# OpenVVC/VVCSoftware_VTM

Hardware: AMD Instinct MI355X
Metric: encoded frames/sec (bit-exact bitstream) at 4K10 RA QP32, 1/2/4/8 GPU [M1: hot-path pictures/s of the kernels behind the call sites, NOT EncoderApp fps] (higher is better)
Workload: dtype int16

## Files before the change

### vvcsoftware_vtm_amd/csrc/fracsearch.hip

```cpp
#include "common.h"
#include "mfma_tr.h"
#include "frac_dev.h"

namespace {

__global__ __launch_bounds__(256) void frac_refine_kernel(const Pel* __restrict__ org, int os, const Pel* __restrict__ ref, int rs,
                                                          const vvcgpu_frac_blk* __restrict__ blocks, int nblocks, int w, int h,
                                                          int bd, int cmin, int cmax, int useHad, vvcgpu_mvcost mv,
                                                          const int* __restrict__ preds, int groups,
                                                          int groupBytes, vvcgpu_frac_result* __restrict__ results)
{
  extern __shared__ __align__(16) unsigned char smem[];
  const int gsz = 256 / groups, grp = threadIdx.x / gsz, tid = threadIdx.x - grp * gsz;
  const int b = blockIdx.x * groups + grp;
  const bool active = b < nblocks;
  const int wp = w + 9 + 1;
  const int WR = h + 9;
  unsigned char* base = smem + (size_t)grp * groupBytes;
  FracLds L;
  L.cost = reinterpret_cast<unsigned long long*>(base);
  L.sel = reinterpret_cast<int*>(base + 512);
  L.org = reinterpret_cast<short*>(base + 544);
  L.win = L.org + ((w * h + 7) & ~7);
  L.hpl = L.win + ((wp * WR + 7) & ~7);
  L.pred = L.hpl + ((w * (h + 8) + 7) & ~7);

  vvcgpu_frac_blk blk = { 0, 0, 0, 0, 0, 0 };
  if (active)
  {
    blk = blocks[b];
    if (preds) { mv.pred_hor = preds[2 * b]; mv.pred_ver = preds[2 * b + 1]; }
    const Pel* o = org + (size_t)blk.org_y * os + blk.org_x;
    for (int i = tid; i < w * h; i += gsz) { const int y = i / w, x = i - y * w; L.org[i] = o[(size_t)y * os + x]; }
    const Pel* r0 = ref + (ptrdiff_t)(blk.ref_y - 4) * rs + blk.ref_x - 4;
    for (int i = tid; i < (w + 9) * WR; i += gsz) { const int y = i / (w + 9), x = i - y * (w + 9); L.win[y * wp + x] = r0[(ptrdiff_t)y * rs + x]; }
  }
  frac_refine_pu(L, w, h, wp, bd, cmin, cmax, useHad, mv, blk.mv_x, blk.mv_y, active, tid, gsz, results + (active ? b : 0));
}

template <int CTRL> __device__ __forceinline__ int dpp_mov(int v) { return __builtin_amdgcn_update_dpp(0, v, CTRL, 0xF, 0xF, false); }
constexpr int DPP_XOR1 = 0xB1, DPP_XOR2 = 0x4E, DPP_HALF_MIRROR = 0x141, DPP_ROR8 = 0x128;

template <int CTRL>
__device__ __forceinline__ void had_cross(int (&v)[4], bool upper)
{
#pragma unroll
  for (int j = 0; j < 4; j++) { const int p = dpp_mov<CTRL>(v[j]); v[j] = (upper ? -v[j] : v[j]) + p; }
}

template <bool HAD>
__device__ __forceinline__ unsigned f16_dist(const int (&orgv)[4], const int (&pred)[4], int lane, bool wide)
{
  int d[4];
#pragma unroll
  for (int j = 0; j < 4; j++) d[j] = orgv[j] - pred[j];
  int s;
  if (HAD && wide)
  {
    int v[4] = { d[0] + d[1], d[0] - d[1], d[2] + d[3], d[2] - d[3] };
    { const int a0 = v[0] + v[2], a2 = v[0] - v[2], a1 = v[1] + v[3], a3 = v[1] - v[3]; v[0] = a0; v[1] = a1; v[2] = a2; v[3] = a3; }
    had_cross<DPP_ROR8>(v, (lane & 8) != 0);
    had_cross<DPP_XOR1>(v, (lane & 1) != 0);
    had_cross<DPP_XOR2>(v, (lane & 2) != 0);
#pragma unroll
    for (int j = 0; j < 4; j++)
    {
      int p = __builtin_amdgcn_update_dpp(0, v[j], 0x104, 0xF, 0x5, false);
      p = __builtin_amdgcn_update_dpp(p, v[j], 0x114, 0xF, 0xA, false);
      v[j] = ((lane & 4) ? -v[j] : v[j]) + p;
    }
    s = abs(v[0]) + abs(v[1]) + abs(v[2]) + abs(v[3]);
  }
  else if (HAD)
  {
    const pel2 one = { 1, 1 }, mone = { -1, -1 }, pm = { 1, -1 };
    pel2 q0 = { (short)d[0], (short)d[1] }, q1 = { (short)d[2], (short)d[3] };
    auto rot = [](pel2 v) { const unsigned u = __builtin_bit_cast(unsigned, v); return __builtin_bit_cast(pel2, __builtin_amdgcn_alignbit(u, u, 16)); };
    q0 = rot(q0) + q0 * pm;
    q1 = rot(q1) + q1 * pm;
    { const pel2 a = q0 + q1, b = q0 - q1; q0 = a; q1 = b; }
    auto cross = [&](auto mov, bool upper)
    {
      const pel2 sg = upper ? mone : one;
      q0 = __builtin_bit_cast(pel2, mov(__builtin_bit_cast(int, q0))) + q0 * sg;
      q1 = __builtin_bit_cast(pel2, mov(__builtin_bit_cast(int, q1))) + q1 * sg;
    };
    cross([](int v) { return dpp_mov<DPP_ROR8>(v); }, (lane & 8) != 0);
    cross([](int v) { return dpp_mov<DPP_XOR1>(v); }, (lane & 1) != 0);
    cross([](int v) { return dpp_mov<DPP_XOR2>(v); }, (lane & 2) != 0);
    auto xor4 = [](int v)
    {
      int p = __builtin_amdgcn_update_dpp(0, v, 0x104, 0xF, 0x5, false);
      return __builtin_amdgcn_update_dpp(p, v, 0x114, 0xF, 0xA, false);
    };
    const pel2 a0 = __builtin_elementwise_max(q0, -q0), a1 = __builtin_elementwise_max(q1, -q1);
    const pel2 m0 = __builtin_elementwise_max(a0, __builtin_bit_cast(pel2, xor4(__builtin_bit_cast(int, a0))));
    const pel2 m1 = __builtin_elementwise_max(a1, __builtin_bit_cast(pel2, xor4(__builtin_bit_cast(int, a1))));
    s = (int)m0[0] + (int)m0[1] + (int)m1[0] + (int)m1[1];
  }
  else
    s = abs(d[0]) + abs(d[1]) + abs(d[2]) + abs(d[3]);
  s += dpp_mov<DPP_XOR1>(s); s += dpp_mov<DPP_XOR2>(s); s += dpp_mov<DPP_HALF_MIRROR>(s); s += dpp_mov<DPP_ROR8>(s);
  unsigned t0 = (unsigned)__builtin_amdgcn_readlane(s, 0), t1 = (unsigned)__builtin_amdgcn_readlane(s, 16),
           t2 = (unsigned)__builtin_amdgcn_readlane(s, 32), t3 = (unsigned)__builtin_amdgcn_readlane(s, 48);
  if (HAD) return ((t0 + 2) >> 2) + ((t1 + 2) >> 2) + ((t2 + 2) >> 2) + ((t3 + 2) >> 2);
  return t0 + t1 + t2 + t3;
}

constexpr int HPT = 24;
struct F16Col { unsigned D[6], E[5]; };
__device__ __forceinline__ void f16_load_col(const short* __restrict__ pcT, F16Col& c)
{
  const uint2* q = reinterpret_cast<const uint2*>(pcT);
#pragma unroll
  for (int m = 0; m < 3; m++) { const uint2 v = q[m]; c.D[2 * m] = v.x; c.D[2 * m + 1] = v.y; }
#pragma unroll
  for (int m = 0; m < 5; m++) c.E[m] = __builtin_amdgcn_alignbit(c.D[m + 1], c.D[m], 16);
}

template <int IY>
__device__ __forceinline__ void f16_vert(const F16Col& col, int fy, int headRoom, int cmin, int cmax, int (&out)[4])
{
  if (fy == 0)
  {
#pragma unroll
    for (int yy = 0; yy < 4; yy++)
    {
      const unsigned d = col.D[2 + (yy >> 1)];
      const int v = (yy & 1) ? (int)d >> 16 : (int)(short)(d & 0xFFFF);
      out[yy] = clip3(cmin, cmax, (int)(short)((v + OFFS + (1 << (headRoom - 1))) >> headRoom));
    }
    return;
  }
  const unsigned* cf = reinterpret_cast<const unsigned*>(c_lumaF[fy << 2]);
  const int shift2 = 6 + headRoom, off2 = (1 << (shift2 - 1)) + (OFFS << 6);
  int sum[4] = { off2, off2, off2, off2 };
#pragma unroll
  for (int m = 0; m < 4; m++)
  {
    const pel2 cm = __builtin_bit_cast(pel2, cf[m]);
    if (IY < 0)
    {
      sum[0] = __builtin_amdgcn_sdot2(__builtin_bit_cast(pel2, col.D[m]), cm, sum[0], false);
      sum[1] = __builtin_amdgcn_sdot2(__builtin_bit_cast(pel2, col.E[m]), cm, sum[1], false);
      sum[2] = __builtin_amdgcn_sdot2(__builtin_bit_cast(pel2, col.D[m + 1]), cm, sum[2], false);
      sum[3] = __builtin_amdgcn_sdot2(__builtin_bit_cast(pel2, col.E[m + 1]), cm, sum[3], false);
    }
    else
    {
      sum[0] = __builtin_amdgcn_sdot2(__builtin_bit_cast(pel2, col.E[m]), cm, sum[0], false);
      sum[1] = __builtin_amdgcn_sdot2(__builtin_bit_cast(pel2, col.D[m + 1]), cm, sum[1], false);
      sum[2] = __builtin_amdgcn_sdot2(__builtin_bit_cast(pel2, col.E[m + 1]), cm, sum[2], false);
      sum[3] = __builtin_amdgcn_sdot2(__builtin_bit_cast(pel2, col.D[m + 2]), cm, sum[3], false);
    }
  }
#pragma unroll
  for (int yy = 0; yy < 4; yy++) out[yy] = clip3(cmin, cmax, (int)(short)(sum[yy] >> shift2));
}

template <bool WIDE>
__device__ __forceinline__ void f16_hplane(const short* __restrict__ win, short* __restrict__ hpT, int ix, int fx, int headRoom, int lane)
{
  if (lane < 48)
  {
    const int r = lane >> 1, seg = lane & 1;
    const unsigned* wr = reinterpret_cast<const unsigned*>(win + r * 26 + seg * 8);
    unsigned D[8], E[7];
#pragma unroll
    for (int k = 0; k < 8; k++) D[k] = wr[k];
#pragma unroll
    for (int k = 0; k < 7; k++) E[k] = __builtin_amdgcn_alignbit(D[k + 1], D[k], 16);
    short* o = hpT + (1 + seg * 8) * HPT + r;
    const int shift1 = 6 - headRoom, off1 = -(OFFS << shift1);
    const unsigned* cf = reinterpret_cast<const unsigned*>(c_lumaF[fx << 2]);
    pel2 c2[4];
#pragma unroll
    for (int m = 0; m < 4; m++) c2[m] = __builtin_bit_cast(pel2, cf[m]);
    auto tap8 = [&](int st) -> int
    {
      int sum = off1;
#pragma unroll
      for (int m = 0; m < 4; m++)
        sum = __builtin_amdgcn_sdot2(__builtin_bit_cast(pel2, (st & 1) ? E[(st >> 1) + m] : D[(st >> 1) + m]), c2[m], sum, false);
      return sum >> shift1;
    };
    if (WIDE)
    {
      if (seg == 0)
      {
#pragma unroll
        for (int x = -1; x < 8; x++) o[x * HPT] = (short)tap8(x + 1);
      }
      else
      {
#pragma unroll
        for (int x = 0; x < 8; x++) o[x * HPT] = (short)tap8(x + 1);
      }
    }
    else if (fx == 0)
    {
#pragma unroll
      for (int x = 0; x < 8; x++)
      {
        const unsigned d = D[(x + 4) >> 1];
        const int sv = (x & 1) ? (int)d >> 16 : (int)(short)(d & 0xFFFF);
        o[x * HPT] = (short)((short)(sv << headRoom) - (short)OFFS);
      }
    }
    else if (ix == 0)
    {
#pragma unroll
      for (int x = 0; x < 8; x++) o[x * HPT] = (short)tap8(x + 1);
    }
    else
    {
#pragma unroll
      for (int x = 0; x < 8; x++) o[x * HPT] = (short)tap8(x);
    }
  }
}

#define WAVE_SYNC() do { __builtin_amdgcn_fence(__ATOMIC_ACQ_REL, "wavefront"); __builtin_amdgcn_wave_barrier(); } while (0)

__device__ __forceinline__ int f16_idx(int dx, int dy, bool quarter)
{
  if (dx == 0) return dy == 0 ? 0 : dy < 0 ? 1 : 2;
  if (!quarter) return dx < 0 ? (dy == 0 ? 3 : dy < 0 ? 5 : 7) : (dy == 0 ? 4 : dy < 0 ? 6 : 8);
  return dx < 0 ? (dy < 0 ? 3 : dy == 0 ? 5 : 7) : (dy < 0 ? 4 : dy == 0 ? 6 : 8);
}

__device__ __forceinline__ void f16_best(const unsigned* dist, bool quarter, const vvcgpu_mvcost& mv, int baseX, int baseY, int scale,
                                         int lane, int& bdx, int& bdy, unsigned long long& bcost, unsigned& bdist)
{
  const int li = lane < 9 ? lane : 0;
  const int dx = quarter ? c_refQ[li][0] : c_refH[li][0], dy = quarter ? c_refQ[li][1] : c_refH[li][1];
  const unsigned dl = dist[li];
  unsigned long long c = lane < 9 ? (unsigned long long)dl + mv_cost(mv.lambda, mv.pred_hor, mv.pred_ver, scale, baseX + dx, baseY + dy) : ~0ull;
  int bi = lane;
#pragma unroll
  for (int o = 1; o < 16; o <<= 1)
  {
    const unsigned long long oc = __shfl_xor(c, o);
    const int oi = __shfl_xor(bi, o);
    if (oc < c || (oc == c && oi < bi)) { c = oc; bi = oi; }
  }
  bi = __builtin_amdgcn_readfirstlane(bi);
  bcost = ((unsigned long long)(unsigned)__builtin_amdgcn_readfirstlane((int)(c >> 32)) << 32) | (unsigned)__builtin_amdgcn_readfirstlane((int)c);
  bdx = quarter ? c_refQ[bi][0] : c_refH[bi][0];
  bdy = quarter ? c_refQ[bi][1] : c_refH[bi][1];
  bdist = dist[bi];
}

struct F16Lds { short win[24 * 26]; short hpl[3][24 * 18]; unsigned dist[16]; };

template <bool HAD>
__device__ __forceinline__ void frac16_pu_valu(F16Lds& L, const Pel* __restrict__ org, int os, const Pel* __restrict__ ref, int rs,
                                               const vvcgpu_frac_blk& blk, int b, int bd, int cmin, int cmax, const vvcgpu_mvcost& mv,
                                               vvcgpu_frac_result* __restrict__ results, int lane)
{
  short* win = L.win;
  short* hp0 = L.hpl[0];
  short* hp8 = L.hpl[1];
  short* hpq = L.hpl[2];
  const int t = lane >> 4, x = 8 * (t & 1) + (lane & 7), y0 = 8 * (t >> 1) + 4 * ((lane >> 3) & 1);
  int orgv[4];
  {
    const Pel* o = org + (size_t)(blk.org_y + y0) * os + blk.org_x + x;
#pragma unroll
    for (int j = 0; j < 4; j++) orgv[j] = o[(size_t)j * os];
    const Pel* r0 = ref + (ptrdiff_t)(blk.ref_y - 4) * rs + blk.ref_x - 4;
#pragma unroll
    for (int u = 0; u < 9; u++)
    {
      const int i = lane + 64 * u, r = (i * 2731) >> 16, cc = i - r * 24;
      win[r * 26 + cc] = r0[(ptrdiff_t)r * rs + cc];
    }
  }
  const bool wide = __ballot(min(min(orgv[0], orgv[1]), min(orgv[2], orgv[3])) < cmax - 1023 || max(max(orgv[0], orgv[1]), max(orgv[2], orgv[3])) > cmin + 1023) != 0ull;
  const int headRoom = max(2, 14 - bd);
  WAVE_SYNC();
  f16_hplane<false>(win, hp0, 0, 0, headRoom, lane);
  f16_hplane<true>(win, hp8, 0, 2, headRoom, lane);
  WAVE_SYNC();

  unsigned* dist = L.dist;
  F16Col col;
  int pred[4];
#pragma unroll
  for (int dx = -1; dx <= 1; dx++)
  {
    const short* pc = dx == 0 ? hp0 + ((1 + x) * HPT + y0) : hp8 + ((1 + x + (dx < 0 ? -1 : 0)) * HPT + y0);
    f16_load_col(pc, col);
    f16_vert<0>(col, 0, headRoom, cmin, cmax, pred);  dist[f16_idx(dx, 0, false)] = f16_dist<HAD>(orgv, pred, lane, wide);
    f16_vert<-1>(col, 2, headRoom, cmin, cmax, pred); dist[f16_idx(dx, -1, false)] = f16_dist<HAD>(orgv, pred, lane, wide);
    f16_vert<0>(col, 2, headRoom, cmin, cmax, pred);  dist[f16_idx(dx, 1, false)] = f16_dist<HAD>(orgv, pred, lane, wide);
  }
  int hx, hy;
  unsigned long long costH;
  unsigned distH;
  WAVE_SYNC();
  f16_best(dist, false, mv, blk.mv_x << 1, blk.mv_y << 1, 1, lane, hx, hy, costH, distH);

#pragma unroll
  for (int dx = -1; dx <= 1; dx++)
  {
    const int qx = 2 * hx + dx, ix = qx >> 2, fx = qx & 3;
    const short* pc;
    if (dx == 0) pc = hx == 0 ? hp0 + ((1 + x) * HPT + y0) : hp8 + ((1 + x + (hx < 0 ? -1 : 0)) * HPT + y0);
    else
    {
      WAVE_SYNC();
      f16_hplane<false>(win, hpq, ix, fx, headRoom, lane);
      WAVE_SYNC();
      pc = hpq + ((1 + x) * HPT + y0);
    }
    f16_load_col(pc, col);
#pragma unroll
    for (int dy = -1; dy <= 1; dy++)
    {
      const int ci = f16_idx(dx, dy, true);
      if (dx == 0 && dy == 0) { dist[ci] = distH; continue; }
      const int qy = 2 * hy + dy, iy = qy >> 2, fy = qy & 3;
      if (iy == 0) f16_vert<0>(col, fy, headRoom, cmin, cmax, pred); else f16_vert<-1>(col, fy, headRoom, cmin, cmax, pred);
      dist[ci] = f16_dist<HAD>(orgv, pred, lane, wide);
    }
  }
  int qdx, qdy;
  unsigned long long costQ;
  unsigned distQ;
  WAVE_SYNC();
  f16_best(dist, true, mv, ((blk.mv_x << 1) + hx) << 1, ((blk.mv_y << 1) + hy) << 1, 0, lane, qdx, qdy, costQ, distQ);
  if (lane == 0)
  {
    vvcgpu_frac_result r;
    r.half_x = hx; r.half_y = hy; r.qter_x = qdx; r.qter_y = qdy; r.cost_half = costH; r.cost = costQ;
    results[b] = r;
  }
  WAVE_SYNC();
}

template <bool HAD>
__global__ __launch_bounds__(256) void frac16_kernel(const Pel* __restrict__ org, int os, const Pel* __restrict__ ref, int rs,
                                                     const vvcgpu_frac_blk* __restrict__ blocks, int nblocks, int bd, int cmin, int cmax,
                                                     vvcgpu_mvcost mv, const int* __restrict__ preds,
                                                     vvcgpu_frac_result* __restrict__ results, int nWg, int xcd)
{
  __shared__ __align__(16) F16Lds ldsS[4];
  const int lane = threadIdx.x & 63, wave = threadIdx.x >> 6;
  const int wg = vvc_xcd_index((int)blockIdx.x, nWg, xcd);
  const int b = wg * 4 + wave;
  if (wg < 0 || b >= nblocks) return;
  const vvcgpu_frac_blk blk = blocks[b];
  if (preds) { mv.pred_hor = preds[2 * b]; mv.pred_ver = preds[2 * b + 1]; }
  frac16_pu_valu<HAD>(ldsS[wave], org, os, ref, rs, blk, b, bd, cmin, cmax, mv, results, lane);
}

__device__ __noinline__ void frac16_pu_valu_call(F16Lds* L, const Pel* __restrict__ org, int os, const Pel* __restrict__ ref, int rs,
                                                 const vvcgpu_frac_blk* __restrict__ blocks, int b, int bd, int cmin, int cmax, vvcgpu_mvcost mv, const int* __restrict__ preds,
                                                 vvcgpu_frac_result* __restrict__ results, int lane)
{
  if (preds) { mv.pred_hor = preds[2 * b]; mv.pred_ver = preds[2 * b + 1]; }
  frac16_pu_valu<true>(*L, org, os, ref, rs, blocks[b], b, bd, cmin, cmax, mv, results, lane);
}
constexpr int FM_FB_MAX = 32;

constexpr int FM_MAT = 512;
constexpr int FM_NA = 7, FM_NB = 14;
constexpr int FM_TAB_HALVES = (FM_NA + FM_NB) * FM_MAT;
typedef _Float16 fh2 __attribute__((ext_vector_type(2)));

__host__ __device__ constexpr int fm_ymap(int n) { return (n & 3) | (((n >> 3) & 1) << 2) | (((n >> 2) & 1) << 3); }
__host__ __device__ constexpr int fm_combo(int f, int i) { return f == 0 ? 0 : 1 + (f - 1) * 2 + (i + 1); }
__host__ __device__ constexpr int fm_idx(int dx, int dy, bool quarter)
{
  return dx == 0 ? (dy == 0 ? 0 : dy < 0 ? 1 : 2)
       : !quarter ? (dx < 0 ? (dy == 0 ? 3 : dy < 0 ? 5 : 7) : (dy == 0 ? 4 : dy < 0 ? 6 : 8))
                  : (dx < 0 ? (dy < 0 ? 3 : dy == 0 ? 5 : 7) : (dy < 0 ? 4 : dy == 0 ? 6 : 8));
}

__global__ void fm_build_tables_kernel(_Float16* __restrict__ tab, int shift2)
{
  const int i = blockIdx.x * 256 + threadIdx.x;
  if (i >= FM_TAB_HALVES) return;
  const int mat = i / FM_MAT, lane = (i % FM_MAT) >> 3, e = i & 7, c16 = lane & 15, g = lane >> 4;
  float v = 0.f;
  if (mat < FM_NA)
  {
    const int fx = mat == 0 ? 0 : 1 + ((mat - 1) >> 1), ix = mat == 0 ? 0 : ((mat - 1) & 1) - 1;
    const int t = 8 * g + e - (c16 + ix + 1);
    if (g < 3 && t >= 0 && t <= 7) v = (float)c_lumaF[fx << 2][t];
    const float S = (float)(1 << (12 - shift2));
    if (g == 3 && e == 0) v = 8192.f * S - 65536.f;
    if (g == 3 && e == 1) v = -0.5f * (S - 1.f);
  }
  else
  {
    const int m = mat - FM_NA, cb = m >> 1, ch = m & 1;
    const int fy = cb == 0 ? 0 : 1 + ((cb - 1) >> 1), iy = cb == 0 ? 0 : ((cb - 1) & 1) - 1;
    const int t = 16 * ch + 4 * g + (e & 3) - (fm_ymap(c16) + iy + 1);
    if (t >= 0 && t <= 7) v = (float)c_lumaF[fy << 2][t] * (e >= 4 ? 128.f : 1.f) / (float)(1 << shift2);
    if (ch == 1 && g == 2 && e < 2)
    {
      const float cinB = (float)(-8454144 - 1048576 + (1 << (shift2 - 1)) + (OFFS << 6) + (1024 << shift2)) / (float)(1 << shift2);
      const float p1 = (float)(_Float16)cinB;
      v = e == 0 ? p1 : cinB - p1;
    }
  }
  tab[i] = (_Float16)v;
}

template <int T> __device__ __forceinline__ unsigned fm_sel(unsigned sp0)
{
  if (T == 0) return sp0;
  return (unsigned)__builtin_amdgcn_mov_dpp((int)sp0, 0x120 + (T ? T : 1), 0xF, 0xF, true);
}

struct FmPu
{
  h8 wA[2];
  fh2 o2[2];
};
struct FmK
{
  float magicA;
  unsigned sp0;
  fh2 pmin, pmax, sg;
  h4 hx;
  unsigned m7[2], m8[2], orX[2], orR[2];
};

__device__ __forceinline__ void fm_plane(const _Float16* __restrict__ tabS, int a, const FmPu& pu, const FmK& K, int lane, h8 (&pl)[2])
{
  const h8 tb = *reinterpret_cast<const h8*>(tabS + (a * 64 + lane) * 8);
#pragma unroll
  for (int ch = 0; ch < 2; ch++)
  {
    const f4 acc = __builtin_amdgcn_mfma_f32_16x16x32_f16(pu.wA[ch], tb, f4{ 0.f, 0.f, 0.f, 0.f }, 0, 0, 0);
    unsigned u[4];
#pragma unroll
    for (int j = 0; j < 4; j++) u[j] = __builtin_bit_cast(unsigned, acc[j] + K.magicA);
    const unsigned p01 = __builtin_amdgcn_perm(u[1], u[0], 0x05040100u), p23 = __builtin_amdgcn_perm(u[3], u[2], 0x05040100u);
    uint4 o;
    o.x = (p01 & K.m7[ch]) | K.orX[ch];
    o.y = (p23 & K.m7[ch]) | K.orR[ch];
    o.z = ((p01 >> 7) & K.m8[ch]) | K.orR[ch];
    o.w = ((p23 >> 7) & K.m8[ch]) | K.orR[ch];
    pl[ch] = __builtin_bit_cast(h8, o);
  }
}

typedef float f2v __attribute__((ext_vector_type(2)));
template <int N>
__device__ __forceinline__ void fm_cands(const _Float16* __restrict__ tabS, const int (&cb)[N], const h8 (&pl)[2], const FmPu& pu, const FmK& K, int lane, float (&P)[N])
{
  h8 b0[N], b1[N];
#pragma unroll
  for (int i = 0; i < N; i++)
  {
    b0[i] = *reinterpret_cast<const h8*>(tabS + ((FM_NA + 2 * cb[i]) * 64 + lane) * 8);
    b1[i] = *reinterpret_cast<const h8*>(tabS + ((FM_NA + 2 * cb[i] + 1) * 64 + lane) * 8);
  }
  f4 acc[N];
#pragma unroll
  for (int i = 0; i < N; i++) acc[i] = __builtin_amdgcn_mfma_f32_16x16x32_f16(pl[0], b0[i], f4{ 0.f, 0.f, 0.f, 0.f }, 0, 0, 0);
#pragma unroll
  for (int i = 0; i < N; i++) acc[i] = __builtin_amdgcn_mfma_f32_16x16x32_f16(pl[1], b1[i], acc[i], 0, 0, 0);
  h4 dv[N];
#pragma unroll
  for (int i = 0; i < N; i++)
  {
    fh2 p0 = __builtin_bit_cast(fh2, __builtin_amdgcn_cvt_pkrtz(acc[i][0], acc[i][1])), p1 = __builtin_bit_cast(fh2, __builtin_amdgcn_cvt_pkrtz(acc[i][2], acc[i][3]));
    p0 = __builtin_elementwise_min(__builtin_elementwise_max(p0, K.pmin), K.pmax);
    p1 = __builtin_elementwise_min(__builtin_elementwise_max(p1, K.pmin), K.pmax);
    fh2 d0 = pu.o2[0] - p0, d1 = pu.o2[1] - p1;
    const fh2 q0 = __builtin_bit_cast(fh2, __builtin_amdgcn_mov_dpp(__builtin_bit_cast(int, d0), DPP_ROR8, 0xF, 0xF, true));
    const fh2 q1 = __builtin_bit_cast(fh2, __builtin_amdgcn_mov_dpp(__builtin_bit_cast(int, d1), DPP_ROR8, 0xF, 0xF, true));
    d0 = __builtin_elementwise_fma(d0, K.sg, q0);
    d1 = __builtin_elementwise_fma(d1, K.sg, q1);
    dv[i] = __builtin_shufflevector(d0, d1, 0, 1, 2, 3);
  }
  f4 e[N];
#pragma unroll
  for (int i = 0; i < N; i++) e[i] = __builtin_amdgcn_mfma_f32_16x16x16f16(dv[i], K.hx, f4{ 0.f, 0.f, 0.f, 0.f }, 0, 0, 0);
#pragma unroll
  for (int i = 0; i < N; i++)
  {
    const f2v lo = { e[i][0], e[i][1] }, hi = { e[i][2], e[i][3] };
    const f2v sm = lo + hi, df = lo - hi;
    P[i] = fmaxf(fabsf(sm[0]), fabsf(sm[1])) + fmaxf(fabsf(df[0]), fabsf(df[1]));
  }
}

__device__ __forceinline__ unsigned fm_limbs(float P)
{
  const float hi = floorf(P * (1.f / 2048.f));
  const float lo = __builtin_fmaf(hi, -2048.f, P);
  return __builtin_bit_cast(unsigned, __builtin_amdgcn_cvt_pkrtz(lo, hi));
}
template <int T0, int T1, int T2>
__device__ __forceinline__ f4 fm_acc(f4 R, float P0, float P1, float P2, const FmK& K)
{
  uint4 a, b;
  a.x = fm_limbs(P0); b.x = fm_sel<T0 & 7>(K.sp0);
  a.y = T1 >= 0 ? fm_limbs(P1) : 0u; b.y = T1 >= 0 ? fm_sel<T1 & 7>(K.sp0) : 0u;
  a.z = T2 >= 0 ? fm_limbs(P2) : 0u; b.z = T2 >= 0 ? fm_sel<T2 & 7>(K.sp0) : 0u;
  a.w = 0u; b.w = 0u;
  return __builtin_amdgcn_mfma_f32_16x16x32_f16(__builtin_bit_cast(h8, a), __builtin_bit_cast(h8, b), R, 0, 0, 0);
}

__device__ __forceinline__ float fm_finalize(const f4& R1, int lane)
{
  const float rr = (R1[0] + R1[1]) + (R1[2] + R1[3]);
  const float col = rr + __builtin_bit_cast(float, __builtin_amdgcn_ds_swizzle(__builtin_bit_cast(int, rr), 0x401F));
  const float sat = floorf((col + 1.f) * 0.5f);
  float s = sat + __builtin_bit_cast(float, __builtin_amdgcn_ds_bpermute((lane ^ 32) << 2, __builtin_bit_cast(int, sat)));
  s += __builtin_bit_cast(float, __builtin_amdgcn_mov_dpp(__builtin_bit_cast(int, s), DPP_ROR8, 0xF, 0xF, true));
  return s;
}

__device__ __forceinline__ unsigned fm_eg_bits(int v)
{
  const unsigned t = (v <= 0) ? ((unsigned)(-v) << 1) + 1 : (unsigned)(v << 1);
  const unsigned k = (unsigned)(t > 128u) + (unsigned)((t >> 7) > 128u) + (unsigned)((t >> 14) > 128u) + (unsigned)((t >> 21) > 128u);
  const unsigned tf = t >> (7 * k);
  return 1 + 14 * k + ((31 - __clz((int)tf)) << 1);
}
constexpr int FM_COST_N = 160;
constexpr unsigned FM_HX = 1u | 1u << 2 | 1u << 4 | 0u << 6 | 2u << 8 | 0u << 10 | 2u << 12 | 0u << 14 | 2u << 16;
constexpr unsigned FM_HY = 1u | 0u << 2 | 2u << 4 | 1u << 6 | 1u << 8 | 0u << 10 | 0u << 12 | 2u << 14 | 2u << 16;
constexpr unsigned FM_QX = 1u | 1u << 2 | 1u << 4 | 0u << 6 | 2u << 8 | 0u << 10 | 2u << 12 | 0u << 14 | 2u << 16;
constexpr unsigned FM_QY = 1u | 0u << 2 | 2u << 4 | 0u << 6 | 0u << 8 | 1u << 10 | 1u << 12 | 2u << 14 | 2u << 16;

__device__ __forceinline__ void fm_best(unsigned dl, bool quarter, const unsigned long long* __restrict__ costS, double lambda, int predH, int predV, int baseX, int baseY, int scale,
                                        int lane, int& bdx, int& bdy, unsigned long long& bcost, unsigned& bdist)
{
  const int li = lane < 9 ? lane : 0;
  const int dx = (int)(((quarter ? FM_QX : FM_HX) >> (2 * li)) & 3u) - 1, dy = (int)(((quarter ? FM_QY : FM_HY) >> (2 * li)) & 3u) - 1;
  const unsigned bits = fm_eg_bits(((baseX + dx) << scale) - predH) + fm_eg_bits(((baseY + dy) << scale) - predV);
  const unsigned long long mc = bits < (unsigned)FM_COST_N ? costS[bits] : (unsigned long long)(lambda * (double)bits);
  unsigned long long c = lane < 9 ? (unsigned long long)dl + mc : ~0ull;
  int bi;
  if (__ballot(lane < 9 && (c >> 32) != 0) == 0ull)
  {
    unsigned m = (unsigned)c;
    m = min(m, (unsigned)__builtin_amdgcn_mov_dpp((int)m, DPP_XOR1, 0xF, 0xF, true));
    m = min(m, (unsigned)__builtin_amdgcn_mov_dpp((int)m, DPP_XOR2, 0xF, 0xF, true));
    m = min(m, (unsigned)__builtin_amdgcn_mov_dpp((int)m, DPP_HALF_MIRROR, 0xF, 0xF, true));
    m = min(m, (unsigned)__builtin_amdgcn_mov_dpp((int)m, 0x140, 0xF, 0xF, true));
    const unsigned m0 = (unsigned)__builtin_amdgcn_readfirstlane((int)m);
    bi = __builtin_ctzll(__ballot((unsigned)c == m0 && lane < 9));
    bcost = m0;
  }
  else
  {
    bi = lane;
#pragma unroll
    for (int o = 1; o < 16; o <<= 1)
    {
      const unsigned long long oc = __shfl_xor(c, o);
      const int oi = __shfl_xor(bi, o);
      if (oc < c || (oc == c && oi < bi)) { c = oc; bi = oi; }
    }
    bi = __builtin_amdgcn_readfirstlane(bi);
    bcost = ((unsigned long long)(unsigned)__builtin_amdgcn_readfirstlane((int)(c >> 32)) << 32) | (unsigned)__builtin_amdgcn_readfirstlane((int)c);
  }
  bdx = (int)(((quarter ? FM_QX : FM_HX) >> (2 * bi)) & 3u) - 1;
  bdy = (int)(((quarter ? FM_QY : FM_HY) >> (2 * bi)) & 3u) - 1;
  bdist = (unsigned)__builtin_amdgcn_readlane((int)dl, bi);
}


template <int WPS, int WV>
__global__ __launch_bounds__(64 * WV, WV == 16 ? 1 : WPS) void frac16m_kernel(const Pel* __restrict__ org, int os, const Pel* __restrict__ ref, int rs,
                                                      const vvcgpu_frac_blk* __restrict__ blocks, int nblocks, int bd, int cmin, int cmax,
                                                      vvcgpu_mvcost mv0, const int* __restrict__ preds,
                                                      vvcgpu_frac_result* __restrict__ results, const _Float16* __restrict__ image,
                                                      int nWg, int xcd)
{
  __shared__ __align__(16) _Float16 tabS[FM_TAB_HALVES];
  __shared__ __align__(16) F16Lds ldsV[WV];
  __shared__ int fbk[WV][FM_FB_MAX];
  int nFb = 0;
  __shared__ unsigned long long costS[FM_COST_N];
  const int wg = vvc_xcd_index((int)blockIdx.x, nWg, xcd);
  if (wg < 0) return;
  for (int i = threadIdx.x; i < FM_TAB_HALVES / 8; i += 64 * WV) reinterpret_cast<uint4*>(tabS)[i] = reinterpret_cast<const uint4*>(image)[i];
  if (threadIdx.x < FM_COST_N) costS[threadIdx.x] = (unsigned long long)(mv0.lambda * (double)threadIdx.x);
  __syncthreads();
  const int lane = threadIdx.x & 63, wave = __builtin_amdgcn_readfirstlane((int)threadIdx.x >> 6), c16 = lane & 15, g = lane >> 4;
  const int headRoom = max(2, 14 - bd), shift1 = 6 - headRoom, S = 1 << shift1;
  FmK K;
  K.magicA = 8388608.f * (float)S;
  K.sp0 = c16 == 8 * (g & 1) ? 0x68003C00u : 0u;
  K.pmin = fh2{ (_Float16)(short)(1024 + cmin), (_Float16)(short)(1024 + cmin) };
  K.pmax = fh2{ (_Float16)(short)(1024 + cmax), (_Float16)(short)(1024 + cmax) };
  K.sg = (c16 & 8) ? fh2{ (_Float16)-1.f, (_Float16)-1.f } : fh2{ (_Float16)1.f, (_Float16)1.f };
#pragma unroll
  for (int j = 0; j < 4; j++)
  {
    const int k = 4 * g + j;
    K.hx[j] = (c16 >> 3) != (k >> 3) ? (_Float16)0.f : (__popc((c16 & 7) & (k & 7)) & 1) ? (_Float16)-1.f : (_Float16)1.f;
  }
  K.m7[0] = 0x007F007Fu; K.m8[0] = 0x00FF00FFu; K.orX[0] = K.orR[0] = 0x64006400u;
  asm("" : "+v"(K.m7[0]), "+v"(K.m8[0]), "+v"(K.orX[0]));
  K.orR[0] = K.orX[0];
  K.m7[1] = g < 2 ? 0x007F007Fu : 0u; K.m8[1] = g < 2 ? 0x00FF00FFu : 0u;
  K.orX[1] = g < 2 ? 0x64006400u : g == 2 ? 0x3C003C00u : 0u; K.orR[1] = g < 2 ? 0x64006400u : 0u;
  const unsigned winAnd = g == 3 ? 0u : 0xFFFFFFFFu, winOrX = g == 3 ? 0x3C003C00u : 0x64006400u, winOrR = g == 3 ? 0u : 0x64006400u;
  const unsigned rangeMask = (unsigned)((1 << bd) - 1) * 0x10001u;
  const int orgLo = max(cmax - 1023, -1024), orgHi = min(cmin + 1023, 1023);
  const int yrow = fm_ymap(c16);
  const int stride = nWg * WV;

  struct Raw { uint4 w[2]; pel4 o; };
  auto fetch = [&](const vvcgpu_frac_blk& blk, Raw& r)
  {
    const Pel* r0 = ref + (ptrdiff_t)(blk.ref_y - 4) * rs + blk.ref_x - 4;
#pragma unroll
    for (int ch = 0; ch < 2; ch++)
    {
      const Pel* q = r0 + (ptrdiff_t)min(16 * ch + c16, 23) * rs + 8 * min(g, 2);
      pel8 v;
#pragma unroll
      for (int e = 0; e < 8; e++) v[e] = q[e];
      r.w[ch] = __builtin_bit_cast(uint4, v);
    }
    const Pel* o = org + (size_t)(blk.org_y + yrow) * os + blk.org_x + 4 * g;
#pragma unroll
    for (int j = 0; j < 4; j++) r.o[j] = o[j];
  };

  int b = wg * WV + wave;
  if (b >= nblocks) return;
  vvcgpu_frac_blk blk = blocks[b];
  int predHN = preds ? preds[2 * b] : mv0.pred_hor, predVN = preds ? preds[2 * b + 1] : mv0.pred_ver;
  Raw raw;
  fetch(blk, raw);
  for (; b < nblocks; b += stride)
  {
    const int bn = b + stride < nblocks ? b + stride : b;
    const uint2* bq = reinterpret_cast<const uint2*>(blocks + bn);
    const uint2 bv0 = bq[0], bv1 = bq[1], bv2 = bq[2];
    const int2 pv = preds ? *reinterpret_cast<const int2*>(preds + 2 * bn) : make_int2(mv0.pred_hor, mv0.pred_ver);
    Raw rawN;
    const int predH = predHN, predV = predVN;
    FmPu pu;
    unsigned bad = 0;
#pragma unroll
    for (int ch = 0; ch < 2; ch++)
    {
      uint4 u = raw.w[ch];
      bad |= (u.x | u.y | u.z | u.w) & ~rangeMask;
      u.x = (u.x & winAnd) | winOrX; u.y = (u.y & winAnd) | winOrR; u.z = (u.z & winAnd) | winOrR; u.w = (u.w & winAnd) | winOrR;
      pu.wA[ch] = __builtin_bit_cast(h8, u);
    }
    {
      const pel4 ov = raw.o;
      const int omin = min(min((int)ov[0], (int)ov[1]), min((int)ov[2], (int)ov[3])), omax = max(max((int)ov[0], (int)ov[1]), max((int)ov[2], (int)ov[3]));
      bad |= (omin < orgLo || omax > orgHi) ? 1u : 0u;
      pu.o2[0] = fh2{ (_Float16)(short)(ov[0] + 1024), (_Float16)(short)(ov[1] + 1024) };
      pu.o2[1] = fh2{ (_Float16)(short)(ov[2] + 1024), (_Float16)(short)(ov[3] + 1024) };
    }
    vvcgpu_frac_blk blkN;
    blkN.org_x = __builtin_amdgcn_readfirstlane((int)bv0.x); blkN.org_y = __builtin_amdgcn_readfirstlane((int)bv0.y);
    blkN.ref_x = __builtin_amdgcn_readfirstlane((int)bv1.x); blkN.ref_y = __builtin_amdgcn_readfirstlane((int)bv1.y);
    blkN.mv_x = __builtin_amdgcn_readfirstlane((int)bv2.x); blkN.mv_y = __builtin_amdgcn_readfirstlane((int)bv2.y);
    predHN = __builtin_amdgcn_readfirstlane(pv.x); predVN = __builtin_amdgcn_readfirstlane(pv.y);
    const bool fallBack = __ballot(bad != 0) != 0ull;
    if (fallBack)
    {
      fetch(blkN, rawN);
      if (lane == 0) fbk[wave][nFb] = b;
      nFb++;
    }
    else
    {
      h8 pl[2];
      f4 Ra = { 0.f, 0.f, 0.f, 0.f }, Rb = { 0.f, 0.f, 0.f, 0.f };
      const int cbH[3] = { fm_combo(0, 0), fm_combo(2, -1), fm_combo(2, 0) };
      float P[3];
      fm_plane(tabS, fm_combo(0, 0), pu, K, lane, pl);
      fm_cands<3>(tabS, cbH, pl, pu, K, lane, P);
      Ra = fm_acc<fm_idx(0, 0, false), fm_idx(0, -1, false), fm_idx(0, 1, false)>(Ra, P[0], P[1], P[2], K);
      fm_plane(tabS, fm_combo(2, -1), pu, K, lane, pl);
      fm_cands<3>(tabS, cbH, pl, pu, K, lane, P);
      Ra = fm_acc<fm_idx(-1, 0, false), fm_idx(-1, -1, false), fm_idx(-1, 1, false)>(Ra, P[0], P[1], P[2], K);
      fetch(blkN, rawN);
      fm_plane(tabS, fm_combo(2, 0), pu, K, lane, pl);
      fm_cands<3>(tabS, cbH, pl, pu, K, lane, P);
      Ra = fm_acc<fm_idx(1, 0, false), fm_idx(1, -1, false), -1>(Ra, P[0], P[1], 0.f, K);
      Rb = fm_acc<fm_idx(1, 1, false), -1, -1>(Rb, P[2], 0.f, 0.f, K);
      const float da = fm_finalize(Ra, lane), db = fm_finalize(Rb, lane);
      int hx, hy;
      unsigned long long costH;
      unsigned distH;
      fm_best((unsigned)(lane == 8 ? db : da), false, costS, mv0.lambda, predH, predV, blk.mv_x << 1, blk.mv_y << 1, 1, lane, hx, hy, costH, distH);

      f4 Rq = { 0.f, 0.f, 0.f, 0.f };
      const int qy0 = 2 * hy - 1, qy1 = 2 * hy, qy2 = 2 * hy + 1;
      const int cb0 = fm_combo(qy0 & 3, (qy0 & 3) ? qy0 >> 2 : 0), cb1 = fm_combo(qy1 & 3, (qy1 & 3) ? qy1 >> 2 : 0), cb2 = fm_combo(qy2 & 3, (qy2 & 3) ? qy2 >> 2 : 0);
      const int cbQ[3] = { cb0, cb1, cb2 }, cbQ2[2] = { cb0, cb2 };
      {
        const int qx = 2 * hx - 1;
        fm_plane(tabS, fm_combo(qx & 3, (qx & 3) ? qx >> 2 : 0), pu, K, lane, pl);
        fm_cands<3>(tabS, cbQ, pl, pu, K, lane, P);
        Rq = fm_acc<fm_idx(-1, -1, true), fm_idx(-1, 0, true), fm_idx(-1, 1, true)>(Rq, P[0], P[1], P[2], K);
      }
      {
        const int qx = 2 * hx;
        float P2[2];
        fm_plane(tabS, fm_combo(qx & 3, (qx & 3) ? qx >> 2 : 0), pu, K, lane, pl);
        fm_cands<2>(tabS, cbQ2, pl, pu, K, lane, P2);
        Rq = fm_acc<fm_idx(0, -1, true), fm_idx(0, 1, true), -1>(Rq, P2[0], P2[1], 0.f, K);
      }
      {
        const int qx = 2 * hx + 1;
        fm_plane(tabS, fm_combo(qx & 3, (qx & 3) ? qx >> 2 : 0), pu, K, lane, pl);
        fm_cands<3>(tabS, cbQ, pl, pu, K, lane, P);
        Rq = fm_acc<fm_idx(1, -1, true), fm_idx(1, 0, true), fm_idx(1, 1, true)>(Rq, P[0], P[1], P[2], K);
      }
      const float dq = fm_finalize(Rq, lane);
      int qdx, qdy;
      unsigned long long costQ;
      unsigned distQ;
      fm_best(lane == 0 ? distH : (unsigned)dq, true, costS, mv0.lambda, predH, predV, ((blk.mv_x << 1) + hx) << 1, ((blk.mv_y << 1) + hy) << 1, 0, lane, qdx, qdy, costQ, distQ);
      if (lane == 0)
      {
        vvcgpu_frac_result r;
        r.half_x = hx; r.half_y = hy; r.qter_x = qdx; r.qter_y = qdy; r.cost_half = costH; r.cost = costQ;
        results[b] = r;
      }
    }
    blk = blkN;
    raw = rawN;
  }
  for (int i = 0; i < nFb; i++)
    frac16_pu_valu_call(&ldsV[wave], org, os, ref, rs, blocks, __builtin_amdgcn_readfirstlane(fbk[wave][i]), bd, cmin, cmax, mv0, preds, results, lane);
}

int fm_build(void* dst, const void* bd)
{
  const int b = *static_cast<const int*>(bd);
  hipLaunchKernelGGL(fm_build_tables_kernel, dim3(cdiv(FM_TAB_HALVES, 256)), dim3(256), 0, (hipStream_t)0, static_cast<_Float16*>(dst), 6 + (14 - b > 2 ? 14 - b : 2));
  VVC_LAUNCH_CHECK();
  return VVCGPU_OK;
}
const _Float16* fm_image(int bd)
{
  void* p = nullptr;
  return vvcgpu_device_image(VVC_IMAGE_FRAC + bd - 8, FM_TAB_HALVES * sizeof(_Float16), fm_build, &bd, &p) == VVCGPU_OK ? static_cast<const _Float16*>(p) : nullptr;
}
}

__attribute__((visibility("hidden"))) int vvcgpu_frac_image_build(int bit_depth) { return fm_image(bit_depth) ? VVCGPU_OK : VVCGPU_E_DEVICE; }

int vvcgpu_frac_refine_launch(const vvc_pel* org, int org_stride, const vvc_pel* ref, int ref_stride,
                              const vvcgpu_frac_blk* blocks, int nblocks, int w, int h, int bit_depth, int clp_min,
                              int clp_max, int use_hadamard, const vvcgpu_mvcost* mvcost_host, const int* preds,
                              vvcgpu_frac_result* results, void* stream)
{
  VVC_CHECK_ARG(nblocks >= 0, "frac_refine: nblocks %d", nblocks);
  if (nblocks == 0) return VVCGPU_OK;
  VVC_CHECK_ARG(org && ref && blocks && mvcost_host && results, "frac_refine: null pointer");
  VVC_CHECK_ARG(w >= 4 && w <= 128 && h >= 4 && h <= 128 && (w & 3) == 0 && (h & 3) == 0, "frac_refine: block %dx%d unsupported", w, h);
  if (bit_depth < 8 || bit_depth > 10) { vvcgpu_set_error("frac_refine: bit depth %d outside 8..10", bit_depth); return VVCGPU_E_UNSUPPORTED; }
  const int wp = w + 10, WR = h + 9;
  auto al8 = [](size_t v) { return (v + 7) & ~(size_t)7; };
  const size_t shorts = al8((size_t)w * h) + al8((size_t)wp * WR) + al8((size_t)w * (h + 8)) + al8((size_t)w * h);
  const size_t groupBytes = (544 + shorts * 2 + 15) & ~(size_t)15;
  const int groups = (w * h <= 1024) ? 4 : 1;
  const size_t smem = groupBytes * groups;
  VVC_CHECK_ARG(smem <= 160 * 1024, "frac_refine: LDS need %zu too large", smem);
  hipStream_t st = (hipStream_t)stream;
  if (w == 16 && h == 16)
  {
    const int xcd = vvc_xcd_on();
    if (use_hadamard && !vvcgpu_no_mfma())
    {
      const _Float16* image = fm_image(bit_depth);
      if (!image) return VVCGPU_E_DEVICE;
      const int cap = 256 * 4;
      for (int first = 0; first < nblocks; first += cap * 4 * FM_FB_MAX)
      {
        const int nb = nblocks - first < cap * 4 * FM_FB_MAX ? nblocks - first : cap * 4 * FM_FB_MAX;
        if (nb >= cap * 4)
        {
          const int nWg = cap / 4;
          hipLaunchKernelGGL((frac16m_kernel<4, 16>), dim3(vvc_xcd_grid(nWg, xcd)), dim3(1024), 0, st, org, org_stride, ref, ref_stride, blocks + first, nb,
                             bit_depth, clp_min, clp_max, *mvcost_host, preds ? preds + 2 * first : nullptr, results + first, image, nWg, xcd);
        }
        else
        {
          const int nWg = cdiv(nb, 4);
          hipLaunchKernelGGL((frac16m_kernel<4, 4>), dim3(vvc_xcd_grid(nWg, xcd)), dim3(256), 0, st, org, org_stride, ref, ref_stride, blocks + first, nb,
                             bit_depth, clp_min, clp_max, *mvcost_host, preds ? preds + 2 * first : nullptr, results + first, image, nWg, xcd);
        }
      }
    }
    else if (use_hadamard)
      hipLaunchKernelGGL(frac16_kernel<true>, dim3(vvc_xcd_grid(cdiv(nblocks, 4), xcd)), dim3(256), 0, st, org, org_stride, ref, ref_stride, blocks, nblocks,
                         bit_depth, clp_min, clp_max, *mvcost_host, preds, results, cdiv(nblocks, 4), xcd);
    else
      hipLaunchKernelGGL(frac16_kernel<false>, dim3(vvc_xcd_grid(cdiv(nblocks, 4), xcd)), dim3(256), 0, st, org, org_stride, ref, ref_stride, blocks, nblocks,
                         bit_depth, clp_min, clp_max, *mvcost_host, preds, results, cdiv(nblocks, 4), xcd);
    VVC_LAUNCH_CHECK();
    return VVCGPU_OK;
  }
  VVC_HIP(vvc_allow_lds(frac_refine_kernel, smem));
  hipLaunchKernelGGL(frac_refine_kernel, dim3(cdiv(nblocks, groups)), dim3(256), smem, st, org, org_stride, ref, ref_stride, blocks,
                     nblocks, w, h, bit_depth, clp_min, clp_max, use_hadamard, *mvcost_host, preds, groups, (int)groupBytes, results);
  VVC_LAUNCH_CHECK();
  return VVCGPU_OK;
}

extern "C" int vvcgpu_frac_refine(const vvc_pel* org, int org_stride, const vvc_pel* ref, int ref_stride,
                                  const vvcgpu_frac_blk* blocks, int nblocks, int w, int h, int bit_depth, int clp_min,
                                  int clp_max, int use_hadamard, const vvcgpu_mvcost* mvcost_host,
                                  vvcgpu_frac_result* results, void* stream)
{
  return vvcgpu_frac_refine_launch(org, org_stride, ref, ref_stride, blocks, nblocks, w, h, bit_depth, clp_min, clp_max, use_hadamard,
                                   mvcost_host, nullptr, results, stream);
}
```

Measured before the change: 2054.

## Use biased-float limb split and pack four candidates per MFMA accumulate

Replaces the floor/fma limb split with a magic-number float add plus a byte permute, and compensates the bias in the finalize step. Candidate limbs are buffered and accumulated four per MFMA instead of three, which cuts the number of matrix ops per half and quarter search. The Exp-Golomb bit count becomes a single clz-based formula, and a few ballots switch to the wave64 builtin. It relies on exact bias cancellation and a changed scale constant for bit-exactness, so the reassociated float sums carry a precision risk.

```diff
diff --git a/vvcsoftware_vtm_amd/csrc/fracsearch.hip b/vvcsoftware_vtm_amd/csrc/fracsearch.hip
--- a/vvcsoftware_vtm_amd/csrc/fracsearch.hip
+++ b/vvcsoftware_vtm_amd/csrc/fracsearch.hip
@@ -491,39 +491,38 @@
   }
 }
 
+constexpr float FM_LIMB_BIAS = 1792.f * 257.f;
 __device__ __forceinline__ unsigned fm_limbs(float P)
 {
-  const float hi = floorf(P * (1.f / 2048.f));
-  const float lo = __builtin_fmaf(hi, -2048.f, P);
-  return __builtin_bit_cast(unsigned, __builtin_amdgcn_cvt_pkrtz(lo, hi));
-}
-template <int T0, int T1, int T2>
-__device__ __forceinline__ f4 fm_acc(f4 R, float P0, float P1, float P2, const FmK& K)
+  const unsigned x = __builtin_bit_cast(unsigned, P + 8388608.f);
+  return __builtin_amdgcn_perm(x, x, 0x03010300u);
+}
+template <int T0, int T1, int T2, int T3>
+__device__ __forceinline__ f4 fm_acc(f4 R, unsigned L0, unsigned L1, unsigned L2, unsigned L3, const FmK& K)
 {
   uint4 a, b;
-  a.x = fm_limbs(P0); b.x = fm_sel<T0 & 7>(K.sp0);
-  a.y = T1 >= 0 ? fm_limbs(P1) : 0u; b.y = T1 >= 0 ? fm_sel<T1 & 7>(K.sp0) : 0u;
-  a.z = T2 >= 0 ? fm_limbs(P2) : 0u; b.z = T2 >= 0 ? fm_sel<T2 & 7>(K.sp0) : 0u;
-  a.w = 0u; b.w = 0u;
+  a.x = L0; b.x = fm_sel<T0 & 7>(K.sp0);
+  a.y = T1 >= 0 ? L1 : 0u; b.y = T1 >= 0 ? fm_sel<T1 & 7>(K.sp0) : 0u;
+  a.z = T2 >= 0 ? L2 : 0u; b.z = T2 >= 0 ? fm_sel<T2 & 7>(K.sp0) : 0u;
+  a.w = T3 >= 0 ? L3 : 0u; b.w = T3 >= 0 ? fm_sel<T3 & 7>(K.sp0) : 0u;
   return __builtin_amdgcn_mfma_f32_16x16x32_f16(__builtin_bit_cast(h8, a), __builtin_bit_cast(h8, b), R, 0, 0, 0);
 }
 
 __device__ __forceinline__ float fm_finalize(const f4& R1, int lane)
 {
-  const float rr = (R1[0] + R1[1]) + (R1[2] + R1[3]);
+  const float rr = ((R1[0] + R1[1]) + R1[2]) + R1[3];
   const float col = rr + __builtin_bit_cast(float, __builtin_amdgcn_ds_swizzle(__builtin_bit_cast(int, rr), 0x401F));
-  const float sat = floorf((col + 1.f) * 0.5f);
+  const float sat = floorf((col + (1.f - 16.f * FM_LIMB_BIAS)) * 0.5f);
   float s = sat + __builtin_bit_cast(float, __builtin_amdgcn_ds_bpermute((lane ^ 32) << 2, __builtin_bit_cast(int, sat)));
   s += __builtin_bit_cast(float, __builtin_amdgcn_mov_dpp(__builtin_bit_cast(int, s), DPP_ROR8, 0xF, 0xF, true));
   return s;
 }
 
-__device__ __forceinline__ unsigned fm_eg_bits(int v)
-{
-  const unsigned t = (v <= 0) ? ((unsigned)(-v) << 1) + 1 : (unsigned)(v << 1);
-  const unsigned k = (unsigned)(t > 128u) + (unsigned)((t >> 7) > 128u) + (unsigned)((t >> 14) > 128u) + (unsigned)((t >> 21) > 128u);
-  const unsigned tf = t >> (7 * k);
-  return 1 + 14 * k + ((31 - __clz((int)tf)) << 1);
+__device__ __forceinline__ unsigned fm_eg_clz(int v)
+{
+  const unsigned w = (unsigned)v << 1;
+  const unsigned t = (v <= 0) ? 1u - w : w;
+  return (unsigned)__builtin_clz(t);
 }
 constexpr int FM_COST_N = 160;
 constexpr unsigned FM_HX = 1u | 1u << 2 | 1u << 4 | 0u << 6 | 2u << 8 | 0u << 10 | 2u << 12 | 0u << 14 | 2u << 16;
@@ -536,11 +535,11 @@
 {
   const int li = lane < 9 ? lane : 0;
   const int dx = (int)(((quarter ? FM_QX : FM_HX) >> (2 * li)) & 3u) - 1, dy = (int)(((quarter ? FM_QY : FM_HY) >> (2 * li)) & 3u) - 1;
-  const unsigned bits = fm_eg_bits(((baseX + dx) << scale) - predH) + fm_eg_bits(((baseY + dy) << scale) - predV);
+  const unsigned bits = 126u - ((fm_eg_clz(((baseX + dx) << scale) - predH) + fm_eg_clz(((baseY + dy) << scale) - predV)) << 1);
   const unsigned long long mc = bits < (unsigned)FM_COST_N ? costS[bits] : (unsigned long long)(lambda * (double)bits);
-  unsigned long long c = lane < 9 ? (unsigned long long)dl + mc : ~0ull;
+  unsigned long long c = lane < 9 ? (unsigned long long)dl + mc : 0xFFFFFFFFull;
   int bi;
-  if (__ballot(lane < 9 && (c >> 32) != 0) == 0ull)
+  if (__builtin_amdgcn_ballot_w64((unsigned)(c >> 32) != 0u) == 0ull)
   {
     unsigned m = (unsigned)c;
     m = min(m, (unsigned)__builtin_amdgcn_mov_dpp((int)m, DPP_XOR1, 0xF, 0xF, true));
@@ -548,11 +547,12 @@
     m = min(m, (unsigned)__builtin_amdgcn_mov_dpp((int)m, DPP_HALF_MIRROR, 0xF, 0xF, true));
     m = min(m, (unsigned)__builtin_amdgcn_mov_dpp((int)m, 0x140, 0xF, 0xF, true));
     const unsigned m0 = (unsigned)__builtin_amdgcn_readfirstlane((int)m);
-    bi = __builtin_ctzll(__ballot((unsigned)c == m0 && lane < 9));
+    bi = __builtin_ctzll(__builtin_amdgcn_ballot_w64((unsigned)c == m0 && lane < 9));
     bcost = m0;
   }
   else
   {
+    if (lane >= 9) c = ~0ull;
     bi = lane;
 #pragma unroll
     for (int o = 1; o < 16; o <<= 1)
@@ -591,7 +591,7 @@
   const int headRoom = max(2, 14 - bd), shift1 = 6 - headRoom, S = 1 << shift1;
   FmK K;
   K.magicA = 8388608.f * (float)S;
-  K.sp0 = c16 == 8 * (g & 1) ? 0x68003C00u : 0u;
+  K.sp0 = c16 == 8 * (g & 1) ? 0x78005800u : 0u;
   K.pmin = fh2{ (_Float16)(short)(1024 + cmin), (_Float16)(short)(1024 + cmin) };
   K.pmax = fh2{ (_Float16)(short)(1024 + cmax), (_Float16)(short)(1024 + cmax) };
   K.sg = (c16 & 8) ? fh2{ (_Float16)-1.f, (_Float16)-1.f } : fh2{ (_Float16)1.f, (_Float16)1.f };
@@ -606,7 +606,8 @@
   K.orR[0] = K.orX[0];
   K.m7[1] = g < 2 ? 0x007F007Fu : 0u; K.m8[1] = g < 2 ? 0x00FF00FFu : 0u;
   K.orX[1] = g < 2 ? 0x64006400u : g == 2 ? 0x3C003C00u : 0u; K.orR[1] = g < 2 ? 0x64006400u : 0u;
-  const unsigned winAnd = g == 3 ? 0u : 0xFFFFFFFFu, winOrX = g == 3 ? 0x3C003C00u : 0x64006400u, winOrR = g == 3 ? 0u : 0x64006400u;
+  unsigned winAnd = g == 3 ? 0u : 0xFFFFFFFFu, winOrX = g == 3 ? 0x3C003C00u : 0x64006400u, winOrR = g == 3 ? 0u : 0x64006400u;
+  asm("" : "+v"(winAnd), "+v"(winOrX), "+v"(winOrR));
   const unsigned rangeMask = (unsigned)((1 << bd) - 1) * 0x10001u;
   const int orgLo = max(cmax - 1023, -1024), orgHi = min(cmin + 1023, 1023);
   const int yrow = fm_ymap(c16);
@@ -666,7 +667,7 @@
     blkN.ref_x = __builtin_amdgcn_readfirstlane((int)bv1.x); blkN.ref_y = __builtin_amdgcn_readfirstlane((int)bv1.y);
     blkN.mv_x = __builtin_amdgcn_readfirstlane((int)bv2.x); blkN.mv_y = __builtin_amdgcn_readfirstlane((int)bv2.y);
     predHN = __builtin_amdgcn_readfirstlane(pv.x); predVN = __builtin_amdgcn_readfirstlane(pv.y);
-    const bool fallBack = __ballot(bad != 0) != 0ull;
+    const bool fallBack = __builtin_amdgcn_ballot_w64(bad != 0) != 0ull;
     if (fallBack)
     {
       fetch(blkN, rawN);
@@ -679,17 +680,20 @@
       f4 Ra = { 0.f, 0.f, 0.f, 0.f }, Rb = { 0.f, 0.f, 0.f, 0.f };
       const int cbH[3] = { fm_combo(0, 0), fm_combo(2, -1), fm_combo(2, 0) };
       float P[3];
+      unsigned L[9];
       fm_plane(tabS, fm_combo(0, 0), pu, K, lane, pl);
       fm_cands<3>(tabS, cbH, pl, pu, K, lane, P);
-      Ra = fm_acc<fm_idx(0, 0, false), fm_idx(0, -1, false), fm_idx(0, 1, false)>(Ra, P[0], P[1], P[2], K);
+      L[fm_idx(0, 0, false)] = fm_limbs(P[0]); L[fm_idx(0, -1, false)] = fm_limbs(P[1]); L[fm_idx(0, 1, false)] = fm_limbs(P[2]);
       fm_plane(tabS, fm_combo(2, -1), pu, K, lane, pl);
       fm_cands<3>(tabS, cbH, pl, pu, K, lane, P);
-      Ra = fm_acc<fm_idx(-1, 0, false), fm_idx(-1, -1, false), fm_idx(-1, 1, false)>(Ra, P[0], P[1], P[2], K);
+      L[fm_idx(-1, 0, false)] = fm_limbs(P[0]); L[fm_idx(-1, -1, false)] = fm_limbs(P[1]); L[fm_idx(-1, 1, false)] = fm_limbs(P[2]);
+      Ra = fm_acc<0, 1, 2, 3>(Ra, L[0], L[1], L[2], L[3], K);
       fetch(blkN, rawN);
       fm_plane(tabS, fm_combo(2, 0), pu, K, lane, pl);
       fm_cands<3>(tabS, cbH, pl, pu, K, lane, P);
-      Ra = fm_acc<fm_idx(1, 0, false), fm_idx(1, -1, false), -1>(Ra, P[0], P[1], 0.f, K);
-      Rb = fm_acc<fm_idx(1, 1, false), -1, -1>(Rb, P[2], 0.f, 0.f, K);
+      L[fm_idx(1, 0, false)] = fm_limbs(P[0]); L[fm_idx(1, -1, false)] = fm_limbs(P[1]); L[fm_idx(1, 1, false)] = fm_limbs(P[2]);
+      Ra = fm_acc<4, 5, 6, 7>(Ra, L[4], L[5], L[6], L[7], K);
+      Rb = fm_acc<8, -1, -1, -1>(Rb, L[8], 0u, 0u, 0u, K);
       const float da = fm_finalize(Ra, lane), db = fm_finalize(Rb, lane);
       int hx, hy;
       unsigned long long costH;
@@ -704,20 +708,22 @@
         const int qx = 2 * hx - 1;
         fm_plane(tabS, fm_combo(qx & 3, (qx & 3) ? qx >> 2 : 0), pu, K, lane, pl);
         fm_cands<3>(tabS, cbQ, pl, pu, K, lane, P);
-        Rq = fm_acc<fm_idx(-1, -1, true), fm_idx(-1, 0, true), fm_idx(-1, 1, true)>(Rq, P[0], P[1], P[2], K);
+        L[fm_idx(-1, -1, true)] = fm_limbs(P[0]); L[fm_idx(-1, 0, true)] = fm_limbs(P[1]); L[fm_idx(-1, 1, true)] = fm_limbs(P[2]);
       }
       {
         const int qx = 2 * hx;
         float P2[2];
         fm_plane(tabS, fm_combo(qx & 3, (qx & 3) ? qx >> 2 : 0), pu, K, lane, pl);
         fm_cands<2>(tabS, cbQ2, pl, pu, K, lane, P2);
-        Rq = fm_acc<fm_idx(0, -1, true), fm_idx(0, 1, true), -1>(Rq, P2[0], P2[1], 0.f, K);
+        L[fm_idx(0, -1, true)] = fm_limbs(P2[0]); L[fm_idx(0, 1, true)] = fm_limbs(P2[1]);
+        Rq = fm_acc<1, 2, 3, 5>(Rq, L[1], L[2], L[3], L[5], K);
       }
       {
         const int qx = 2 * hx + 1;
         fm_plane(tabS, fm_combo(qx & 3, (qx & 3) ? qx >> 2 : 0), pu, K, lane, pl);
         fm_cands<3>(tabS, cbQ, pl, pu, K, lane, P);
-        Rq = fm_acc<fm_idx(1, -1, true), fm_idx(1, 0, true), fm_idx(1, 1, true)>(Rq, P[0], P[1], P[2], K);
+        L[fm_idx(1, -1, true)] = fm_limbs(P[0]); L[fm_idx(1, 0, true)] = fm_limbs(P[1]); L[fm_idx(1, 1, true)] = fm_limbs(P[2]);
+        Rq = fm_acc<4, 6, 7, 8>(Rq, L[4], L[6], L[7], L[8], K);
       }
       const float dq = fm_finalize(Rq, lane);
       int qdx, qdy;
```

Result: faster. 2081, median of 6 (+1.3%).
